# itmo153277/JoshUpscale

Hardware: AMD Instinct MI355X
Metric: frames/sec 480x270->1920x1080 recurrent SR (higher is better)
Workload: dtype bf16

## Files before the change

### joshupscale_amd/csrc/flow_kernels.hip

```cpp
#include "flow_block_common.h"

namespace ju {

namespace {

struct FlowBlockParams {
	const void *in;
	const void *w1;
	const float *b1;
	const void *w2;
	const float *b2;
	void *out;
	int H, W;
	int inPitch, outPitch;
	int act1, act2;
	float slope;
	int skip;
	int prio;
	const void *packPrev;
	void *packOut;
	int frameH, frameW, padTop, padLeft, numInputs;
	const unsigned *sums;
	long inItem, outItem;
	const std::uint8_t *frames[kFlowBatchMax];
	std::ptrdiff_t frameStrides[kFlowBatchMax];
	const void *packPrevs[kFlowBatchMax];
	void *packOuts[kFlowBatchMax];
	const int *cutAt;
};

template <int CIN, int CMID, int TH, bool UPS, bool POOL, int OUTK, int NW = 4>
struct FbGeom {
	static constexpr int CK1 = CIN >= 64 ? 64 : CIN;
	static constexpr int NPL = CIN / CK1;
	static constexpr int PBX = CK1 * 2;
	static constexpr int KS1 = CK1 / 16;
	static constexpr int XR = TH + 4;
	static constexpr int TR = TH + 2;
	static constexpr int XPLANE = XR * kFbW * PBX;
	static constexpr int PBT = CMID * 2;
	static constexpr int KS2 = CMID / 16;
	static constexpr int NCB = CMID / 32;
	static constexpr int TBYTES = TR * kFbW * PBT;
	static constexpr int LR = XR / 2 + 1, LC = kFbW / 2 + 1;
	static constexpr int LBYTES = UPS ? NPL * LR * LC * PBX : 0;
	static constexpr bool XPAIR = UPS && NPL > 2 && TH > 2;
	static constexpr int NPLX = XPAIR ? 2 : NPL;
	static constexpr int OFF_X = 0;
	static constexpr int OFF_T = NPLX * XPLANE;
	static constexpr int TREGION = TBYTES > LBYTES ? TBYTES : LBYTES;
	static constexpr int ESZ = 2;
	static constexpr int RBW = 32 * ESZ;
	static constexpr int STAGE_PX = POOL ? 16 : 64;
	static constexpr int STAGE_WAVE = STAGE_PX * RBW;
	static constexpr bool STAGE_IN_X = NPLX * XPLANE >= NW * STAGE_WAVE;
	static constexpr int OFF_STAGE = STAGE_IN_X ? OFF_X : OFF_T + TREGION;
	static constexpr int LDS = OFF_T + TREGION + (STAGE_IN_X ? 0 : NW * STAGE_WAVE);
	static_assert(CIN == 16 || CIN == 32 || CIN == 64 || CIN == 128 || CIN == 256, "input channels");
#ifndef JU_FB_RELOAD_MIN
#define JU_FB_RELOAD_MIN 3
#endif
	static constexpr bool RELOAD = NPL >= JU_FB_RELOAD_MIN;
	static_assert(CMID == 32 || CMID == 64 || CMID == 128, "block filters");
	static_assert(NW % NCB == 0, "cout blocks over the waves");
	static_assert(TH % 2 == 0 && TH >= 2, "row pairs");
	static constexpr bool FITS = LDS <= 160 * 1024;
};

template <typename T, int CIN, int CMID, int TH, bool UPS, bool POOL, int OUTK, int NW, bool PACK = false, bool INDEP = false,
    bool CUT = false>
__global__ __launch_bounds__(NW * 64, NW / 4) void flow_block_kernel(FlowBlockParams p) {
	static_assert(!PACK || (CIN == 16 && !UPS), "PACK: the 16-channel flow input");
	static_assert(!INDEP || PACK, "INDEP: a form of the input packing");
	static_assert(!CUT || (PACK && !INDEP), "CUT: a form of the look-ahead input packing");
	using G = FbGeom<CIN, CMID, TH, UPS, POOL, OUTK, NW>;
	constexpr int NT = NW * 64;
	extern __shared__ __attribute__((aligned(16))) unsigned char smem[];
	const int tid = threadIdx.x;
	const int wave = tid >> 6;
	if constexpr (NW == 8) applyWavePriority(p.prio, wave, NW);
	const int lane = tid & 63;
	const int px = lane & 31;
	const int hh = lane >> 5;
	const int x0 = blockIdx.x * kFbOutW;
	const int y0 = blockIdx.y * TH;
	const int item = blockIdx.z;
	const T *__restrict__ in = reinterpret_cast<const T *>(static_cast<const unsigned char *>(p.in) + item * p.inItem);
	const unsigned ldsBase = static_cast<unsigned>(reinterpret_cast<unsigned long long>(
	    (__attribute__((address_space(3))) unsigned char *)smem));

	constexpr int NCB = G::NCB;
	const int cb = wave % NCB;
	const int pstart = wave / NCB;
	constexpr int PSTEP = NW / NCB;
	const float s1 = fbActS(p.act1, p.slope), s2 = fbActS(p.act2, p.slope);

	constexpr int NWA = G::RELOAD ? ((NW == 4 && !G::XPAIR) ? 2 : 1) : G::NPL;
	Vec8<T> wa[NWA][9 * G::KS1];
	const unsigned char *waSrc = static_cast<const unsigned char *>(p.w1) +
	                             (size_t)cb * G::NPL * (9 * G::KS1 * 1024) + lane * 16;
	auto loadPlaneA = [&](int set, int pl) __attribute__((always_inline)) {
#pragma unroll
		for (int f = 0; f < 9 * G::KS1; ++f) {
			wa[set][f] = *reinterpret_cast<const Vec8<T> *>(waSrc + (size_t)(pl * 9 * G::KS1 + f) * 1024);
		}
	};
	if constexpr (G::RELOAD) {
		loadPlaneA(0, 0);
	} else {
#pragma unroll
		for (int pl = 0; pl < G::NPL; ++pl) loadPlaneA(pl, pl);
	}

	[[maybe_unused]] constexpr int LPPX = G::PBX / 16;
	[[maybe_unused]] auto expandPlanes = [&](int plFirst, int plCount) __attribute__((always_inline)) {
		if constexpr (UPS) {
			constexpr int LPP = LPPX;
			constexpr int NPIX = G::LR * G::LC;
			const unsigned char *smL = smem + G::OFF_T;
			constexpr int BR = G::XR / 2, BC = kFbW / 2;
			const int nel = plCount * BR * BC * LPP;
			for (int e = tid; e < nel; e += NT) {
				const int c = e % LPP;
				const int bq = (e / LPP) % (BR * BC);
				const int pl = plFirst + e / (LPP * BR * BC);
				const int br = bq / BC, bc = bq - br * BC;
				const unsigned char *base = smL + pl * (NPIX * G::PBX) + (br * G::LC + bc) * G::PBX + c * 16;
				const Vec8<T> tl = *reinterpret_cast<const Vec8<T> *>(base);
				const Vec8<T> tr = *reinterpret_cast<const Vec8<T> *>(base + G::PBX);
				const Vec8<T> bl = *reinterpret_cast<const Vec8<T> *>(base + G::LC * G::PBX);
				const Vec8<T> brr = *reinterpret_cast<const Vec8<T> *>(base + (G::LC + 1) * G::PBX);
				Vec8<T> o01, o10, o11;
#pragma unroll
				for (int j = 0; j < 8; ++j) {
					const float a = static_cast<float>(tl[j]), b2 = static_cast<float>(tr[j]);
					const float d = static_cast<float>(bl[j]), e2 = static_cast<float>(brr[j]);
					const float top = a + (b2 - a) * 0.5f;
					const float bot = d + (e2 - d) * 0.5f;
					o01[j] = static_cast<T>(top);
					o10[j] = static_cast<T>(a + (d - a) * 0.5f);
					o11[j] = static_cast<T>(top + (bot - top) * 0.5f);
				}
				const int r = 2 * br, k = 2 * bc;
				const int gy = y0 - 2 + r, gx = x0 - 2 + k;
				const Vec8<T> zero = {static_cast<T>(0.f), static_cast<T>(0.f), static_cast<T>(0.f), static_cast<T>(0.f),
				    static_cast<T>(0.f), static_cast<T>(0.f), static_cast<T>(0.f), static_cast<T>(0.f)};
				const bool inside = gy >= 0 && gy < p.H && gx >= 0 && gx < p.W;
				unsigned char *xb = smem + G::OFF_X + (G::XPAIR ? (pl & 1) : pl) * G::XPLANE + (r * kFbW + k) * G::PBX;
				const unsigned s0 = (static_cast<unsigned>(c) ^ fbSwz<G::PBX>(k)) << 4;
				const unsigned s1x = (static_cast<unsigned>(c) ^ fbSwz<G::PBX>(k + 1)) << 4;
				*reinterpret_cast<Vec8<T> *>(xb + s0) = inside ? tl : zero;
				*reinterpret_cast<Vec8<T> *>(xb + G::PBX + s1x) = inside ? o01 : zero;
				*reinterpret_cast<Vec8<T> *>(xb + kFbW * G::PBX + s0) = inside ? o10 : zero;
				*reinterpret_cast<Vec8<T> *>(xb + (kFbW + 1) * G::PBX + s1x) = inside ? o11 : zero;
			}
		}
	};
	const bool border = y0 - 2 < 0 || y0 + TH + 2 > p.H || x0 - 2 < 0 || x0 + 32 > p.W;
	constexpr int LPP = G::PBX / 16;
	if (JU_SKIP(p) & 1) {
	} else if constexpr (PACK) {
		const float bright = brightnessOf(p.sums, 1.0f / static_cast<float>(p.frameH * p.frameW));
		const T *__restrict__ prev = static_cast<const T *>(INDEP ? p.packPrevs[item] : p.packPrev);
		T *__restrict__ cur = INDEP ? static_cast<T *>(p.packOuts[item])
		                            : (item + 1 == static_cast<int>(gridDim.z) ? static_cast<T *>(p.packOut) : nullptr);
		const int nch = 3 * p.numInputs;
		int fromFrames = INDEP ? 1 : min(item + 1, p.numInputs);
		[[maybe_unused]] bool fromPrev = true;
		if constexpr (CUT) {
			const int c = p.cutAt[item];
			if (c >= 0) {
				fromFrames = min(item - c + 1, p.numInputs);
				fromPrev = false;
			}
		}
		constexpr int NPIX = G::XR * kFbW;
		for (int q = tid; q < NPIX; q += NT) {
			const int r = q / kFbW, k = q - r * kFbW;
			const int gy = y0 - 2 + r, gx = x0 - 2 + k;
			const T zero = static_cast<T>(0.f);
			Vec8<T> o0 = {zero, zero, zero, zero, zero, zero, zero, zero}, o1 = o0;
			const bool inside = gy >= 0 && gy < p.H && gx >= 0 && gx < p.W;
			if (inside) {
				const int y = gy - p.padTop, x = gx - p.padLeft;
				const bool inFrame = y >= 0 && y < p.frameH && x >= 0 && x < p.frameW;
				const size_t idx = (size_t)gy * p.W + gx;
				T pv[16], o[16];
#pragma unroll
				for (int j = 0; j < 16; ++j) o[j] = zero;
#pragma unroll
				for (int h = 0; h < 5; ++h) {
					if (h < fromFrames) {
						float c0 = 0.f, c1 = 0.f, c2 = 0.f;
						if (inFrame) {
							const unsigned v = *reinterpret_cast<const unsigned *>(p.frames[item - h] + y * p.frameStrides[item - h] + x * 4);
							c0 = preprocessU8(v & 0xff) - bright;
							c1 = preprocessU8((v >> 8) & 0xff) - bright;
							c2 = preprocessU8((v >> 16) & 0xff) - bright;
						}
						o[3 * h] = static_cast<T>(c0);
						o[3 * h + 1] = static_cast<T>(c1);
						o[3 * h + 2] = static_cast<T>(c2);
					}
				}
				if (fromFrames < p.numInputs && (!CUT || fromPrev)) {
					const Vec8<T> p0 = *reinterpret_cast<const Vec8<T> *>(prev + idx * 16);
					const Vec8<T> p1 = *reinterpret_cast<const Vec8<T> *>(prev + idx * 16 + 8);
#pragma unroll
					for (int i = 0; i < 8; ++i) {
						pv[i] = p0[i];
						pv[8 + i] = p1[i];
					}
					auto shifted = [&](auto sTag) __attribute__((always_inline)) {
						constexpr int S = decltype(sTag)::value;
#pragma unroll
						for (int j = S; j < 16; ++j) o[j] = (j < nch) ? pv[j - S] : zero;
					};
					if (fromFrames == 1) shifted(std::integral_constant<int, 3>{});
					else if (fromFrames == 2) shifted(std::integral_constant<int, 6>{});
					else if (fromFrames == 3) shifted(std::integral_constant<int, 9>{});
					else shifted(std::integral_constant<int, 12>{});
				}
#pragma unroll
				for (int i = 0; i < 8; ++i) {
					o0[i] = o[i];
					o1[i] = o[8 + i];
				}
				if (cur != nullptr && r >= 2 && r < 2 + TH && k >= 2 && k < 2 + kFbOutW) {
					*reinterpret_cast<Vec8<T> *>(cur + idx * 16) = o0;
					*reinterpret_cast<Vec8<T> *>(cur + idx * 16 + 8) = o1;
				}
			}
			unsigned char *xb = smem + G::OFF_X + (r * kFbW + k) * G::PBX;
			const unsigned sw = fbSwz<G::PBX>(k);
			*reinterpret_cast<Vec8<T> *>(xb + ((0u ^ sw) << 4)) = o0;
			*reinterpret_cast<Vec8<T> *>(xb + ((1u ^ sw) << 4)) = o1;
		}
		__syncthreads();
	} else if constexpr (!UPS) {
		if (border) {
			for (int i = tid; i < G::NPL * G::XPLANE / 16; i += NT) {
				reinterpret_cast<uint4 *>(smem + G::OFF_X)[i] = make_uint4(0, 0, 0, 0);
			}
			__syncthreads();
		}
		constexpr int NPXI = 1024 / G::PBX;
		constexpr int NPIX = G::XR * kFbW;
		constexpr int NINSTR = (NPIX + NPXI - 1) / NPXI;
#pragma unroll
		for (int pl = 0; pl < G::NPL; ++pl) {
			for (int i = wave; i < NINSTR; i += NW) {
				const int q = i * NPXI + lane / LPP;
				const int r = q / kFbW, k = q - r * kFbW;
				const int gy = y0 - 2 + r, gx = x0 - 2 + k;
				const unsigned c = static_cast<unsigned>(lane % LPP) ^ fbSwz<G::PBX>(k);
				if (q < NPIX && gy >= 0 && gy < p.H && gx >= 0 && gx < p.W) {
					fbGlds16(in + ((size_t)gy * p.inPitch + gx) * CIN + pl * 64 + c * 8,
					    smem + G::OFF_X + pl * G::XPLANE + i * 1024);
				}
			}
		}
		asm volatile("s_waitcnt vmcnt(0)" ::: "memory");
		__syncthreads();
	} else {
		unsigned char *smL = smem + G::OFF_T;
		const int lh = p.H >> 1, lw = p.W >> 1;
		const int ly0 = (y0 >> 1) - 1, lx0 = (x0 >> 1) - 1;
		constexpr int NPXI = 1024 / G::PBX;
		constexpr int NPIX = G::LR * G::LC;
		constexpr int NINSTR = (NPIX + NPXI - 1) / NPXI;
#pragma unroll
		for (int pl = 0; pl < G::NPL; ++pl) {
			for (int i = wave; i < NINSTR; i += NW) {
				const int q = min(i * NPXI + lane / LPP, NPIX - 1);
				const int r = q / G::LC, k = q - r * G::LC;
				const int cy = min(max(ly0 + r, 0), lh - 1), cx = min(max(lx0 + k, 0), lw - 1);
				if (i * NPXI + lane / LPP < NPIX) {
					fbGlds16(in + ((size_t)cy * p.inPitch + cx) * CIN + pl * 64 + (lane % LPP) * 8,
					    smL + pl * (NPIX * G::PBX) + i * 1024);
				}
			}
		}
		asm volatile("s_waitcnt vmcnt(0)" ::: "memory");
		__syncthreads();
		if constexpr (!G::XPAIR) {
			expandPlanes(0, G::NPL);
		} else {
			expandPlanes(0, 1);
		}
		__syncthreads();
	}

	unsigned colOffA[3], colSwzA[3];
#pragma unroll
	for (int dx = 0; dx < 3; ++dx) {
		colOffA[dx] = (px + dx) * G::PBX;
		colSwzA[dx] = fbSwz<G::PBX>(px + dx);
	}
	{
		constexpr int NPAIR = G::TR / 2;
		constexpr int MAXP = (NPAIR + PSTEP - 1) / PSTEP;
		constexpr int HOLD = G::NPL > 1 ? MAXP : 1;
		f32x16 acc[HOLD][2];
		unsigned tOff[4];
#pragma unroll
		for (int g = 0; g < 4; ++g) {
			tOff[g] = px * G::PBT + ((static_cast<unsigned>(cb * 4 + g) ^ fbSwz<G::PBT>(px)) << 4) + hh * 8;
		}
		constexpr bool kHoistBiasA = NWA * 9 * G::KS1 * 4 < 144 || NW == 4;
		f32x4 biasA[4];
		if constexpr (kHoistBiasA) {
#pragma unroll
			for (int g = 0; g < 4; ++g) biasA[g] = *reinterpret_cast<const f32x4 *>(p.b1 + cb * 32 + 8 * g + 4 * hh);
		}
		auto initAcc = [&](f32x16(&a)[2]) {
#pragma unroll
			for (int g = 0; g < 4; ++g) {
				f32x4 bg;
				if constexpr (kHoistBiasA) bg = biasA[g];
				else bg = *reinterpret_cast<const f32x4 *>(p.b1 + cb * 32 + 8 * g + 4 * hh);
#pragma unroll
				for (int r = 0; r < 2; ++r) {
#pragma unroll
					for (int i = 0; i < 4; ++i) a[r][4 * g + i] = bg[i];
				}
			}
		};
		auto epilogueA = [&](const f32x16(&a)[2], int pair) {
			const int gx = x0 - 1 + px;
			const bool colIn = gx >= 0 && gx < p.W;
#pragma unroll
			for (int r = 0; r < 2; ++r) {
				const int tr = 2 * pair + r;
				const int gy = y0 - 1 + tr;
				const float keep = (colIn && gy >= 0 && gy < p.H) ? 1.0f : 0.0f;
				unsigned char *row = smem + G::OFF_T + tr * (kFbW * G::PBT);
#pragma unroll
				for (int g = 0; g < 4; ++g) {
					*reinterpret_cast<Vec4<T> *>(row + tOff[g]) =
					    pack4<T>(fbAct(a[r][4 * g + 0], s1) * keep, fbAct(a[r][4 * g + 1], s1) * keep,
					        fbAct(a[r][4 * g + 2], s1) * keep, fbAct(a[r][4 * g + 3], s1) * keep);
				}
			}
		};
		if (JU_SKIP(p) & 2) {
		} else if constexpr (G::NPL == 1) {
			for (int pair = pstart; pair < NPAIR; pair += PSTEP) {
				initAcc(acc[0]);
				FbPair<T, G::KS1, G::PBX>::run(ldsBase + G::OFF_X + (2 * pair) * (kFbW * G::PBX), colOffA, colSwzA,
				    hh, wa[0], acc[0]);
				epilogueA(acc[0], pair);
			}
		} else {
#pragma unroll
			for (int s = 0; s < HOLD; ++s) initAcc(acc[s]);
#pragma unroll
			for (int pl = 0; pl < G::NPL; ++pl) {
				if constexpr (G::RELOAD && NWA == 2) {
					if (pl + 1 < G::NPL) loadPlaneA((pl + 1) & 1, pl + 1);
				}
				if constexpr (G::XPAIR) {
					if (pl + 1 < G::NPL && !(JU_SKIP(p) & 1)) expandPlanes(pl + 1, 1);
				}
#pragma unroll
				for (int s = 0; s < HOLD; ++s) {
					const int pair = pstart + s * PSTEP;
					if (pair < NPAIR) {
						FbPair<T, G::KS1, G::PBX>::run(
						    ldsBase + G::OFF_X + (G::XPAIR ? (pl & 1) : pl) * G::XPLANE + (2 * pair) * (kFbW * G::PBX), colOffA,
						    colSwzA, hh, wa[G::RELOAD ? (pl & (NWA - 1)) : pl], acc[s]);
					}
				}
				if constexpr (G::RELOAD && NWA == 1) {
					if (pl + 1 < G::NPL) loadPlaneA(0, pl + 1);
				}
				if constexpr (G::XPAIR) __syncthreads();
			}
#pragma unroll
			for (int s = 0; s < HOLD; ++s) {
				const int pair = pstart + s * PSTEP;
				if (pair < NPAIR) epilogueA(acc[s], pair);
			}
		}
	}

	Vec8<T> wb[9 * G::KS2];
	f32x4 biasB[4];
	{
		const unsigned char *wsrc = static_cast<const unsigned char *>(p.w2) + (size_t)cb * (9 * G::KS2 * 1024) + lane * 16;
#pragma unroll
		for (int f = 0; f < 9 * G::KS2; ++f) {
			constexpr int KSP = G::KS2 > 4 ? 4 : G::KS2;
			const int tap = f / G::KS2, ks = f % G::KS2;
			wb[f] = *reinterpret_cast<const Vec8<T> *>(wsrc + (size_t)(((ks / KSP) * 9 + tap) * KSP + ks % KSP) * 1024);
		}
#pragma unroll
		for (int g = 0; g < 4; ++g) biasB[g] = *reinterpret_cast<const f32x4 *>(p.b2 + cb * 32 + 8 * g + 4 * hh);
	}
	__syncthreads();

	unsigned colOffB[3], colSwzB[3];
#pragma unroll
	for (int dx = 0; dx < 3; ++dx) {
		colOffB[dx] = (px + dx) * G::PBT;
		colSwzB[dx] = fbSwz<G::PBT>(px + dx);
	}
	unsigned char *stage = smem + G::OFF_STAGE + wave * G::STAGE_WAVE;
	constexpr int NCH = G::RBW / 16;
	for (int pair = pstart; pair < ((JU_SKIP(p) & 4) ? 0 : TH / 2); pair += PSTEP) {
		f32x16 acc[2];
#pragma unroll
		for (int g = 0; g < 4; ++g) {
#pragma unroll
			for (int r = 0; r < 2; ++r) {
#pragma unroll
				for (int i = 0; i < 4; ++i) acc[r][4 * g + i] = biasB[g][i];
			}
		}
		FbPair<T, G::KS2, G::PBT>::run(ldsBase + G::OFF_T + (2 * pair) * (kFbW * G::PBT), colOffB, colSwzB, hh, wb, acc);
		Vec4<T> resv[2][4];
		if constexpr (OUTK == 2) {
			static_assert(CIN == CMID && !UPS && !POOL, "residual block: same width in and out");
#pragma unroll
			for (int r = 0; r < 2; ++r) {
				const int gy = min(y0 + 2 * pair + r, p.H - 1), gx = min(x0 + px, p.W - 1);
				const T *rp = in + ((size_t)gy * p.inPitch + gx) * CIN + cb * 32 + 4 * hh;
#pragma unroll
				for (int g = 0; g < 4; ++g) resv[r][g] = *reinterpret_cast<const Vec4<T> *>(rp + 8 * g);
			}
		}
		if constexpr (POOL) {
			const int pp = px >> 1;
#pragma unroll
			for (int g = 0; g < 4; ++g) {
				float v[4];
#pragma unroll
				for (int i = 0; i < 4; ++i) {
					float m = fmaxf(acc[0][4 * g + i], acc[1][4 * g + i]);
					m = fmaxf(m, fbSwapPair(m));
					v[i] = fbAct(m, s2);
				}
				if ((g >> 1) == (px & 1)) {
					const unsigned c = static_cast<unsigned>(g) ^ (static_cast<unsigned>(pp) & (NCH - 1));
					*reinterpret_cast<Vec4<T> *>(stage + pp * G::RBW + (c << 4) + hh * 8) = pack4<T>(v[0], v[1], v[2], v[3]);
				}
			}
		} else {
#pragma unroll
			for (int r = 0; r < 2; ++r) {
				const int pi = r * 32 + px;
#pragma unroll
				for (int g = 0; g < 4; ++g) {
					float v[4];
#pragma unroll
					for (int i = 0; i < 4; ++i) {
						float x = acc[r][4 * g + i];
						if constexpr (OUTK == 2) x += static_cast<float>(resv[r][g][i]);
						v[i] = fbAct(x, s2);
					}
					const unsigned c = static_cast<unsigned>(g) ^ (static_cast<unsigned>(pi) & (NCH - 1));
					if constexpr (OUTK == 1) {
						*reinterpret_cast<Vec4<f16> *>(stage + pi * G::RBW + (c << 4) + hh * 8) = pack4<f16>(v[0], v[1], v[2], v[3]);
					} else {
						*reinterpret_cast<Vec4<T> *>(stage + pi * G::RBW + (c << 4) + hh * 8) = pack4<T>(v[0], v[1], v[2], v[3]);
					}
				}
			}
		}
		__builtin_amdgcn_fence(__ATOMIC_RELEASE, "wavefront");
		__builtin_amdgcn_wave_barrier();
		__builtin_amdgcn_fence(__ATOMIC_ACQUIRE, "wavefront");
		{
			unsigned char *outp = static_cast<unsigned char *>(p.out) + item * p.outItem;
			constexpr int PXI = 64 / NCH;
#pragma unroll
			for (int it = 0; it < G::STAGE_PX / PXI; ++it) {
				const int pi = it * PXI + lane / NCH;
				const unsigned slot = static_cast<unsigned>(lane % NCH);
				const unsigned chunk = slot ^ (static_cast<unsigned>(pi) & (NCH - 1));
				const uint4 val = *reinterpret_cast<const uint4 *>(stage + pi * G::RBW + (slot << 4));
				if (JU_SKIP(p) & 8) {
				} else if constexpr (POOL) {
					const int oy = (y0 >> 1) + pair, ox = (x0 >> 1) + pi;
					if (pi < kFbOutW / 2 && oy < (p.H >> 1) && ox < (p.W >> 1)) {
						*reinterpret_cast<uint4 *>(outp + (((size_t)oy * p.outPitch + ox) * CMID + cb * 32) * G::ESZ + chunk * 16) = val;
					}
				} else {
					const int gy = y0 + 2 * pair + (pi >> 5), gx = x0 + (pi & 31);
					if ((pi & 31) < kFbOutW && gy < p.H && gx < p.W) {
						*reinterpret_cast<uint4 *>(outp + (((size_t)gy * p.outPitch + gx) * CMID + cb * 32) * G::ESZ + chunk * 16) = val;
					}
				}
			}
		}
		__builtin_amdgcn_fence(__ATOMIC_RELEASE, "wavefront");
		__builtin_amdgcn_wave_barrier();
	}
}

template <int CIN, int CMID = 32>
constexpr int fbWaves() {
#if JU_FB_RELOAD_MIN <= 2
	if (CIN == 128 && CMID <= 64) return 8;
#endif
	return (CIN > 64 || CMID > 64) ? 4 : 8;
}

template <typename T, int CIN, int CMID, int TH, bool UPS, bool POOL, int OUTK, bool PACK = false, bool INDEP = false, bool CUT = false>
void launchFlowBlockInst(const FlowBlockParams &p, int items, hipStream_t stream) {
	constexpr int NW = fbWaves<CIN, CMID>();
	using G = FbGeom<CIN, CMID, TH, UPS, POOL, OUTK, NW>;
	static_assert(G::FITS, "tile does not fit LDS");
	auto kern = flow_block_kernel<T, CIN, CMID, TH, UPS, POOL, OUTK, NW, PACK, INDEP, CUT>;
	static std::atomic<std::uint64_t> ldsDone{0};
	ensureDynamicLds(reinterpret_cast<const void *>(kern), G::LDS, &ldsDone, "flow block");
	if (launchesAreDry()) return;
	dim3 grid((p.W + kFbOutW - 1) / kFbOutW, (p.H + TH - 1) / TH, items);
	hipLaunchKernelGGL(kern, grid, dim3(NW * 64), G::LDS, stream, p);
	hipCheckLaunch("flow_block");
}

constexpr int kFbMid = 14;
constexpr int kFbFixedRows = 8;

inline long fbLaunchCost(int H, long tilesX, int TH, int numCUs, int items = 1) {
	const long tiles = tilesX * ((H + TH - 1) / TH) * items;
	return (tiles + numCUs - 1) / numCUs * (TH + kFbFixedRows);
}

void fbNotePlan(const DevPlan *plan, int cin, int cmid, bool ups, bool pool, int outk, bool pack, bool indep, int H, int W,
    int items, int rows, const int *heights, int nHeights) {
	std::string line = "flow_block cin=" + std::to_string(cin) + " cmid=" + std::to_string(cmid) + " ups=" + std::to_string(ups) +
	                   " pool=" + std::to_string(pool) + " outk=" + std::to_string(outk) + " pack=" + std::to_string(pack) +
	                   " indep=" + std::to_string(indep) + " H=" + std::to_string(H) + " W=" + std::to_string(W) +
	                   " items=" + std::to_string(items) + " rows=" + std::to_string(rows) + " heights=";
	for (int i = 0; i < nHeights; ++i) line += (i ? "," : "") + std::to_string(heights[i]);
	plan->log->note(line);
}

template <typename T, int CIN, int CMID, bool UPS, bool POOL, int OUTK, bool PACK, bool INDEP, bool CUT, int... THS>
void launchFlowBlockBest(const FlowBlockParams &p, int items, int numCUs, const DevPlan *plan, hipStream_t stream) {
	const long tilesX = (p.W + kFbOutW - 1) / kFbOutW;
	const int forced = plan ? plan->flowTile : 0;
	int best = 0;
	long bestCost = 0;
	int heights[sizeof...(THS)], nHeights = 0;
	auto consider = [&](int TH, bool fits) {
		if (!fits) return;
		heights[nHeights++] = TH;
		const long c = forced == TH ? -1 : fbLaunchCost(p.H, tilesX, TH, numCUs, items);
		if (best == 0 || c < bestCost) {
			best = TH;
			bestCost = c;
		}
	};
	(consider(THS, FbGeom<CIN, CMID, THS, UPS, POOL, OUTK, fbWaves<CIN, CMID>()>::FITS), ...);
	if (plan && plan->log) fbNotePlan(plan, CIN, CMID, UPS, POOL, OUTK, PACK, INDEP, p.H, p.W, items, best, heights, nHeights);
	bool done = false;
	auto launch = [&](auto thTag) {
		constexpr int TH = decltype(thTag)::value;
		if constexpr (FbGeom<CIN, CMID, TH, UPS, POOL, OUTK, fbWaves<CIN, CMID>()>::FITS) {
			if (!done && best == TH) {
				launchFlowBlockInst<T, CIN, CMID, TH, UPS, POOL, OUTK, PACK, INDEP, CUT>(p, items, stream);
				done = true;
			}
		}
	};
	(launch(std::integral_constant<int, THS>{}), ...);
	if (!done) throw std::logic_error("flow block: no tile height fits");
}

template <typename T, int CIN, int CMID, bool UPS, bool POOL, int OUTK, bool PACK = false, bool INDEP = false, bool CUT = false>
void launchFlowBlockT(const FlowBlockParams &p, int items, int numCUs, const DevPlan *plan, hipStream_t stream) {
	if constexpr (OUTK == 2) {
		launchFlowBlockBest<T, CIN, CMID, UPS, POOL, OUTK, PACK, INDEP, CUT, kFbMid, 6>(p, items, numCUs, plan, stream);
	} else if constexpr (CMID == 128) {
		launchFlowBlockBest<T, CIN, CMID, UPS, POOL, OUTK, PACK, INDEP, CUT, 6, 4, 2>(p, items, numCUs, plan, stream);
	} else {
		launchFlowBlockBest<T, CIN, CMID, UPS, POOL, OUTK, PACK, INDEP, CUT, 20, 18, 10, 6>(p, items, numCUs, plan, stream);
	}
}

template <typename T>
void launchFlowBlockDT(const FlowBlockLaunch &q, hipStream_t stream) {
	FlowBlockParams p{};
	p.in = q.in;
	p.w1 = q.w1;
	p.b1 = q.b1;
	p.w2 = q.w2;
	p.b2 = q.b2;
	p.out = q.out;
	p.H = q.H;
	p.W = q.W;
	p.inPitch = q.inPitch ? q.inPitch : (q.upsample ? q.W / 2 : q.W);
	p.outPitch = q.outPitch ? q.outPitch : (q.pool ? q.W / 2 : q.W);
	p.act1 = q.act1;
	p.act2 = q.act2;
	p.slope = q.slope;
	p.skip = ablationSkipBits();
	p.prio = wavePriorityMode(0);
	p.packPrev = q.packPrev;
	p.packOut = q.packOut;
	p.frameH = q.frameH;
	p.frameW = q.frameW;
	p.padTop = q.padTop;
	p.padLeft = q.padLeft;
	p.numInputs = q.numInputs;
	p.sums = q.sums;
	const int items = q.items > 1 ? q.items : 1;
	if (items > kFlowBatchMax) throw std::invalid_argument("flow block: more look-ahead frames than kFlowBatchMax");
	p.inItem = items > 1 ? q.inItemBytes : 0;
	p.outItem = items > 1 ? q.outItemBytes : 0;
	const bool many = items > 1 || q.independentItems;
	for (int i = 0; i < kFlowBatchMax; ++i) {
		p.frames[i] = many ? (i < items ? q.packFrames[i] : nullptr) : (i == 0 ? q.packFrame : nullptr);
		p.frameStrides[i] = many ? (i < items ? q.packFrameStrides[i] : 0) : (i == 0 ? q.packFrameStride : 0);
		p.packPrevs[i] = q.independentItems && i < items ? q.packPrevs[i] : nullptr;
		p.packOuts[i] = q.independentItems && i < items ? q.packOuts[i] : nullptr;
	}
	if (items > 1 && q.residual) throw std::invalid_argument("flow block: the residual form has no look-ahead launch");
	const int cus = currentDeviceCUs();
	if (q.packOut != nullptr || q.independentItems) {
		if (many && q.sums != nullptr) throw std::invalid_argument("flow block: look-ahead packing has no brightness sums");
		for (int i = 0; i < items; ++i) {
			if (p.frames[i] == nullptr) throw std::invalid_argument("flow block: input packing needs every frame of the launch");
			if (q.independentItems && (p.packPrevs[i] == nullptr || p.packOuts[i] == nullptr)) {
				throw std::invalid_argument("flow block: independent items need every item's history buffers");
			}
		}
		if (!(q.cin == 16 && q.cmid == 32 && !q.upsample && q.pool && !q.outHead && !q.residual &&
		        (q.packPrev || q.independentItems))) {
			throw std::invalid_argument("flow block: input packing is built for the first block (16 -> 32 -> 32, pool)");
		}
		if (q.independentItems) return launchFlowBlockT<T, 16, 32, false, true, 0, true, true>(p, items, cus, q.plan, stream);
		if (q.cutAt != nullptr) {
			if (items < 2) throw std::invalid_argument("flow block: cut-aware history is a form of the look-ahead launch");
			p.cutAt = q.cutAt;
			return launchFlowBlockT<T, 16, 32, false, true, 0, true, false, true>(p, items, cus, q.plan, stream);
		}
		return launchFlowBlockT<T, 16, 32, false, true, 0, true>(p, items, cus, q.plan, stream);
	}
	if (q.upsample && (q.H % 2 || q.W % 2)) throw std::invalid_argument("flow block: fused upsampling needs even H and W");
	if (q.pool && (q.H % 2 || q.W % 2)) throw std::invalid_argument("flow block: fused max-pool needs even H and W");
	const int outk = q.residual ? 2 : (q.outHead ? 1 : 0);
#define JU_FB_CASE(CIN_, CMID_, UPS_, POOL_, OUTK_)                                              \
	if (q.cin == CIN_ && q.cmid == CMID_ && q.upsample == UPS_ && q.pool == POOL_ && outk == OUTK_) { \
		return launchFlowBlockT<T, CIN_, CMID_, UPS_, POOL_, OUTK_>(p, items, cus, q.plan, stream); \
	}
	JU_FB_CASE(16, 32, false, true, 0)
	JU_FB_CASE(32, 64, false, true, 0)
	JU_FB_CASE(64, 128, false, true, 0)
	JU_FB_CASE(256, 128, true, false, 0)
	JU_FB_CASE(256, 128, false, false, 0)
	JU_FB_CASE(128, 64, true, false, 0)
	JU_FB_CASE(128, 64, false, false, 0)
	JU_FB_CASE(64, 32, true, false, 1)
	JU_FB_CASE(64, 32, false, false, 1)
	JU_FB_CASE(64, 64, false, false, 2)
#undef JU_FB_CASE
	throw std::invalid_argument("flow block: unsupported shape");
}

}

bool flowBlockSupported(int cin, int cmid, bool upsample, bool pool, bool outHead, int H, int W) {
	if (cin == 64 && cmid == 64) return false;
	if (cin == 16 && cmid == 32) return !upsample && pool && !outHead;
	if (cin == 32 && cmid == 64) return !upsample && pool && !outHead;
	if (cmid == 128) {
		const char *wideEnv = devSwitch(Dev::FlowWide);
		const int wide = wideEnv ? std::atoi(wideEnv) : 2;
		const int rows = (cin == 256 && !upsample) ? 2 : 6;
		const bool oneRound = H <= 0 || W <= 0 || wide >= 3 ||
		                      static_cast<long>((W + kFbOutW - 1) / kFbOutW) * ((H + rows - 1) / rows) <= currentDeviceCUs();
		if (cin == 64) return wide >= 1 && oneRound && !upsample && pool && !outHead;
		if (cin == 256) return wide >= 2 && oneRound && !pool && !outHead;
		return false;
	}
	if (cin == 128 && cmid == 64) return !pool && !outHead;
	if (cin == 64 && cmid == 32) return !pool && outHead;
	return false;
}

void launchFlowBlock(DType dt, const FlowBlockLaunch &q, hipStream_t stream) {
	if (q.residual && q.cin == 64 && q.cmid == 64 && !q.upsample && !q.pool) {
		if (!(q.plan && q.plan->resBlock == 2)) {
			launchResBlockPersistent(dt, q, stream);
			return;
		}
	}
	if (dt == kF16) launchFlowBlockDT<f16>(q, stream);
	else launchFlowBlockDT<bf16>(q, stream);
}

}
```

Baseline: 2237.

## Expand upsampled flow-block input directly from global memory into registers

Adds a DIRECT mode for upsampling flow blocks that loads the four low-res neighbours straight from global memory into registers, then bilinearly expands and writes to the LDS input tile. This skips the intermediate LDS staging of the low-res tile and its extra barrier. An optional XPIPE form overlaps the next plane's loads with the current plane's MMA work. The default enables DIRECT only for CIN=128. It raises register pressure and issues redundant global loads, since neighbours are fetched four times through cache.

```diff
diff --git a/joshupscale_amd/csrc/flow_kernels.hip b/joshupscale_amd/csrc/flow_kernels.hip
--- a/joshupscale_amd/csrc/flow_kernels.hip
+++ b/joshupscale_amd/csrc/flow_kernels.hip
@@ -29,6 +29,20 @@
 	const int *cutAt;
 };
 
+#ifndef JU_FB_EXPAND_64
+#define JU_FB_EXPAND_64 0
+#endif
+#ifndef JU_FB_EXPAND_128
+#define JU_FB_EXPAND_128 1
+#endif
+#ifndef JU_FB_EXPAND_256
+#define JU_FB_EXPAND_256 0
+#endif
+template <int CIN>
+constexpr int fbExpandForm() {
+	return CIN == 64 ? JU_FB_EXPAND_64 : (CIN == 128 ? JU_FB_EXPAND_128 : (CIN == 256 ? JU_FB_EXPAND_256 : 0));
+}
+
 template <int CIN, int CMID, int TH, bool UPS, bool POOL, int OUTK, int NW = 4>
 struct FbGeom {
 	static constexpr int CK1 = CIN >= 64 ? 64 : CIN;
@@ -43,7 +57,10 @@
 	static constexpr int NCB = CMID / 32;
 	static constexpr int TBYTES = TR * kFbW * PBT;
 	static constexpr int LR = XR / 2 + 1, LC = kFbW / 2 + 1;
-	static constexpr int LBYTES = UPS ? NPL * LR * LC * PBX : 0;
+	static constexpr int XFORM = UPS ? fbExpandForm<CIN>() : 0;
+	static constexpr bool DIRECT = XFORM >= 1;
+	static constexpr bool XPIPE = XFORM == 2 && NPL > 1 && !(NPL > 2 && TH == 2);
+	static constexpr int LBYTES = (UPS && !DIRECT) ? NPL * LR * LC * PBX : 0;
 	static constexpr bool XPAIR = UPS && NPL > 2 && TH > 2;
 	static constexpr int NPLX = XPAIR ? 2 : NPL;
 	static constexpr int OFF_X = 0;
@@ -113,47 +130,92 @@
 	}
 
 	[[maybe_unused]] constexpr int LPPX = G::PBX / 16;
+	[[maybe_unused]] constexpr int XBR = G::XR / 2, XBC = kFbW / 2;
+	[[maybe_unused]] auto expandBlock = [&](int pl, int c, int br, int bc, const Vec8<T> &tl, const Vec8<T> &tr, const Vec8<T> &bl,
+	                                        const Vec8<T> &brr) __attribute__((always_inline)) {
+		Vec8<T> o01, o10, o11;
+#pragma unroll
+		for (int j = 0; j < 8; ++j) {
+			const float a = static_cast<float>(tl[j]), b2 = static_cast<float>(tr[j]);
+			const float d = static_cast<float>(bl[j]), e2 = static_cast<float>(brr[j]);
+			const float top = a + (b2 - a) * 0.5f;
+			const float bot = d + (e2 - d) * 0.5f;
+			o01[j] = static_cast<T>(top);
+			o10[j] = static_cast<T>(a + (d - a) * 0.5f);
+			o11[j] = static_cast<T>(top + (bot - top) * 0.5f);
+		}
+		const int r = 2 * br, k = 2 * bc;
+		const int gy = y0 - 2 + r, gx = x0 - 2 + k;
+		const Vec8<T> zero = {static_cast<T>(0.f), static_cast<T>(0.f), static_cast<T>(0.f), static_cast<T>(0.f),
+		    static_cast<T>(0.f), static_cast<T>(0.f), static_cast<T>(0.f), static_cast<T>(0.f)};
+		const bool inside = gy >= 0 && gy < p.H && gx >= 0 && gx < p.W;
+		unsigned char *xb = smem + G::OFF_X + (G::XPAIR ? (pl & 1) : pl) * G::XPLANE + (r * kFbW + k) * G::PBX;
+		const unsigned s0 = (static_cast<unsigned>(c) ^ fbSwz<G::PBX>(k)) << 4;
+		const unsigned s1x = (static_cast<unsigned>(c) ^ fbSwz<G::PBX>(k + 1)) << 4;
+		*reinterpret_cast<Vec8<T> *>(xb + s0) = inside ? tl : zero;
+		*reinterpret_cast<Vec8<T> *>(xb + G::PBX + s1x) = inside ? o01 : zero;
+		*reinterpret_cast<Vec8<T> *>(xb + kFbW * G::PBX + s0) = inside ? o10 : zero;
+		*reinterpret_cast<Vec8<T> *>(xb + (kFbW + 1) * G::PBX + s1x) = inside ? o11 : zero;
+	};
 	[[maybe_unused]] auto expandPlanes = [&](int plFirst, int plCount) __attribute__((always_inline)) {
-		if constexpr (UPS) {
-			constexpr int LPP = LPPX;
+		if constexpr (UPS && !G::DIRECT) {
 			constexpr int NPIX = G::LR * G::LC;
 			const unsigned char *smL = smem + G::OFF_T;
-			constexpr int BR = G::XR / 2, BC = kFbW / 2;
-			const int nel = plCount * BR * BC * LPP;
+			const int nel = plCount * XBR * XBC * LPPX;
 			for (int e = tid; e < nel; e += NT) {
-				const int c = e % LPP;
-				const int bq = (e / LPP) % (BR * BC);
-				const int pl = plFirst + e / (LPP * BR * BC);
-				const int br = bq / BC, bc = bq - br * BC;
+				const int c = e % LPPX;
+				const int bq = (e / LPPX) % (XBR * XBC);
+				const int pl = plFirst + e / (LPPX * XBR * XBC);
+				const int br = bq / XBC, bc = bq - br * XBC;
 				const unsigned char *base = smL + pl * (NPIX * G::PBX) + (br * G::LC + bc) * G::PBX + c * 16;
-				const Vec8<T> tl = *reinterpret_cast<const Vec8<T> *>(base);
-				const Vec8<T> tr = *reinterpret_cast<const Vec8<T> *>(base + G::PBX);
-				const Vec8<T> bl = *reinterpret_cast<const Vec8<T> *>(base + G::LC * G::PBX);
-				const Vec8<T> brr = *reinterpret_cast<const Vec8<T> *>(base + (G::LC + 1) * G::PBX);
-				Vec8<T> o01, o10, o11;
-#pragma unroll
-				for (int j = 0; j < 8; ++j) {
-					const float a = static_cast<float>(tl[j]), b2 = static_cast<float>(tr[j]);
-					const float d = static_cast<float>(bl[j]), e2 = static_cast<float>(brr[j]);
-					const float top = a + (b2 - a) * 0.5f;
-					const float bot = d + (e2 - d) * 0.5f;
-					o01[j] = static_cast<T>(top);
-					o10[j] = static_cast<T>(a + (d - a) * 0.5f);
-					o11[j] = static_cast<T>(top + (bot - top) * 0.5f);
-				}
-				const int r = 2 * br, k = 2 * bc;
-				const int gy = y0 - 2 + r, gx = x0 - 2 + k;
-				const Vec8<T> zero = {static_cast<T>(0.f), static_cast<T>(0.f), static_cast<T>(0.f), static_cast<T>(0.f),
-				    static_cast<T>(0.f), static_cast<T>(0.f), static_cast<T>(0.f), static_cast<T>(0.f)};
-				const bool inside = gy >= 0 && gy < p.H && gx >= 0 && gx < p.W;
-				unsigned char *xb = smem + G::OFF_X + (G::XPAIR ? (pl & 1) : pl) * G::XPLANE + (r * kFbW + k) * G::PBX;
-				const unsigned s0 = (static_cast<unsigned>(c) ^ fbSwz<G::PBX>(k)) << 4;
-				const unsigned s1x = (static_cast<unsigned>(c) ^ fbSwz<G::PBX>(k + 1)) << 4;
-				*reinterpret_cast<Vec8<T> *>(xb + s0) = inside ? tl : zero;
-				*reinterpret_cast<Vec8<T> *>(xb + G::PBX + s1x) = inside ? o01 : zero;
-				*reinterpret_cast<Vec8<T> *>(xb + kFbW * G::PBX + s0) = inside ? o10 : zero;
-				*reinterpret_cast<Vec8<T> *>(xb + (kFbW + 1) * G::PBX + s1x) = inside ? o11 : zero;
-			}
+				expandBlock(pl, c, br, bc, *reinterpret_cast<const Vec8<T> *>(base), *reinterpret_cast<const Vec8<T> *>(base + G::PBX),
+				    *reinterpret_cast<const Vec8<T> *>(base + G::LC * G::PBX),
+				    *reinterpret_cast<const Vec8<T> *>(base + (G::LC + 1) * G::PBX));
+			}
+		}
+	};
+	constexpr int XPLC = (G::XPIPE || G::XPAIR) ? 1 : G::NPL;
+	constexpr int XPEL = XBR * XBC * LPPX;
+	constexpr int XNEL = XPLC * XPEL;
+	constexpr int XNR = G::DIRECT ? (XNEL + NT - 1) / NT : 1;
+	constexpr int XD = (G::XPIPE || XNR < 4) ? XNR : 4;
+	[[maybe_unused]] Vec8<T> xl[XD][4];
+	[[maybe_unused]] auto expandLoad = [&](int slot, int plFirst, int round) __attribute__((always_inline)) {
+		if constexpr (G::DIRECT) {
+			const int lh = p.H >> 1, lw = p.W >> 1;
+			const int ly0 = (y0 >> 1) - 1, lx0 = (x0 >> 1) - 1;
+			const int e = min(tid + round * NT, XNEL - 1);
+			const int c = e % LPPX, bq = (e / LPPX) % (XBR * XBC), pl = plFirst + e / XPEL;
+			const int br = bq / XBC, bc = bq - br * XBC;
+			const int cy0 = min(max(ly0 + br, 0), lh - 1), cy1 = min(max(ly0 + br + 1, 0), lh - 1);
+			const int cx0 = min(max(lx0 + bc, 0), lw - 1), cx1 = min(max(lx0 + bc + 1, 0), lw - 1);
+			const T *r0 = in + (size_t)cy0 * p.inPitch * CIN + pl * 64 + c * 8;
+			const T *r1 = in + (size_t)cy1 * p.inPitch * CIN + pl * 64 + c * 8;
+			xl[slot][0] = *reinterpret_cast<const Vec8<T> *>(r0 + (size_t)cx0 * CIN);
+			xl[slot][1] = *reinterpret_cast<const Vec8<T> *>(r0 + (size_t)cx1 * CIN);
+			xl[slot][2] = *reinterpret_cast<const Vec8<T> *>(r1 + (size_t)cx0 * CIN);
+			xl[slot][3] = *reinterpret_cast<const Vec8<T> *>(r1 + (size_t)cx1 * CIN);
+		}
+	};
+	[[maybe_unused]] auto expandStore = [&](int slot, int plFirst, int round) __attribute__((always_inline)) {
+		if constexpr (G::DIRECT) {
+			const int e = tid + round * NT;
+			if (e < XNEL) {
+				const int c = e % LPPX, bq = (e / LPPX) % (XBR * XBC), pl = plFirst + e / XPEL;
+				const int br = bq / XBC, bc = bq - br * XBC;
+				expandBlock(pl, c, br, bc, xl[slot][0], xl[slot][1], xl[slot][2], xl[slot][3]);
+			}
+		}
+	};
+	[[maybe_unused]] auto expandIssue = [&](int plFirst) __attribute__((always_inline)) {
+#pragma unroll
+		for (int r = 0; r < XD; ++r) expandLoad(r, plFirst, r);
+	};
+	[[maybe_unused]] auto expandFinish = [&](int plFirst) __attribute__((always_inline)) {
+#pragma unroll
+		for (int r = 0; r < XNR; ++r) {
+			expandStore(r % XD, plFirst, r);
+			if (r + XD < XNR) expandLoad(r % XD, plFirst, r + XD);
 		}
 	};
 	const bool border = y0 - 2 < 0 || y0 + TH + 2 > p.H || x0 - 2 < 0 || x0 + 32 > p.W;
@@ -262,6 +324,10 @@
 		}
 		asm volatile("s_waitcnt vmcnt(0)" ::: "memory");
 		__syncthreads();
+	} else if constexpr (G::DIRECT) {
+		expandIssue(0);
+		expandFinish(0);
+		__syncthreads();
 	} else {
 		unsigned char *smL = smem + G::OFF_T;
 		const int lh = p.H >> 1, lw = p.W >> 1;
@@ -359,8 +425,17 @@
 				if constexpr (G::RELOAD && NWA == 2) {
 					if (pl + 1 < G::NPL) loadPlaneA((pl + 1) & 1, pl + 1);
 				}
-				if constexpr (G::XPAIR) {
-					if (pl + 1 < G::NPL && !(JU_SKIP(p) & 1)) expandPlanes(pl + 1, 1);
+				if constexpr (G::XPIPE) {
+					if (pl + 1 < G::NPL && !(JU_SKIP(p) & 1)) expandIssue(pl + 1);
+				} else if constexpr (G::XPAIR) {
+					if (pl + 1 < G::NPL && !(JU_SKIP(p) & 1)) {
+						if constexpr (G::DIRECT) {
+							expandIssue(pl + 1);
+							expandFinish(pl + 1);
+						} else {
+							expandPlanes(pl + 1, 1);
+						}
+					}
 				}
 #pragma unroll
 				for (int s = 0; s < HOLD; ++s) {
@@ -374,7 +449,14 @@
 				if constexpr (G::RELOAD && NWA == 1) {
 					if (pl + 1 < G::NPL) loadPlaneA(0, pl + 1);
 				}
-				if constexpr (G::XPAIR) __syncthreads();
+				if constexpr (G::XPIPE) {
+					if (pl + 1 < G::NPL) {
+						if (!(JU_SKIP(p) & 1)) expandFinish(pl + 1);
+						__syncthreads();
+					}
+				} else if constexpr (G::XPAIR) {
+					__syncthreads();
+				}
 			}
 #pragma unroll
 			for (int s = 0; s < HOLD; ++s) {
```

Result: no change. 2237, median of 3 (+0.0%).
